# tlk00/BitMagic

Hardware: AMD Instinct MI355X
Metric: Gbits/s + % HBM roofline, 256-way fused AND+COUNT on 1B-bit vectors (higher is better)
Workload: dtype u64; 1 GPU; aggregator pipeline combine_and_sub counts-only: 256-way AND+COUNT, 256 x 1000000000-bit vectors in total, data set A (common 10% OR noise 10%: no early exit); vectors=256, bits_per_vector=1000000000, density_q16=6554, blocks_per_vector=15259, blocks_per_rank=15259, hbm_resident_bytes=32279432448

## Files before the change

bitmagic_amd/csrc/bmx_device.h:

```cpp
#pragma once
#include <hip/hip_runtime.h>
#include <stdint.h>

typedef uint8_t  u8;
typedef uint16_t u16;
typedef uint32_t u32;
typedef uint64_t u64;

#define GMETA(e) ((u32)((e) >> 48) & 0x1FFFu)
#define GMETA_NONE 0xFFFFFFFFu
#define BMX_DESC_KIND(d) ((u32)((d) & 3ull))
#define BMX_DESC_PTR(d)  ((d) & ~3ull)

typedef u32 u32x4 __attribute__((ext_vector_type(4)));
typedef const __attribute__((address_space(1))) u32x4* gcptr4;
typedef __attribute__((address_space(1))) u32x4* gptr4;
typedef const __attribute__((address_space(1))) u16* gcptr16;

template <int ROWS> struct Part { u32x4 r[ROWS]; };
typedef Part<8> Blk;

__device__ __forceinline__ gcptr4 as_gc4(u64 addr) { return (gcptr4)(uintptr_t)addr; }
__device__ __forceinline__ gcptr4 as_gc4(const void* p) { return (gcptr4)(uintptr_t)p; }
__device__ __forceinline__ gptr4 as_g4(void* p) { return (gptr4)(uintptr_t)p; }
__device__ __forceinline__ gcptr16 as_gc16(u64 addr) { return (gcptr16)(uintptr_t)(addr & 0x0000FFFFFFFFFFFFull); }

__device__ __forceinline__ u32 lane_id() { return threadIdx.x & 63u; }

__device__ __forceinline__ u64 uniform64(u64 v)
{
    u32 lo = __builtin_amdgcn_readfirstlane((u32)v);
    u32 hi = __builtin_amdgcn_readfirstlane((u32)(v >> 32));
    return ((u64)hi << 32) | lo;
}
__device__ __forceinline__ u32 uniform32(u32 v) { return __builtin_amdgcn_readfirstlane(v); }

__device__ __forceinline__ u32 wave_sum(u32 v)
{
#pragma unroll
    for (int o = 32; o > 0; o >>= 1) v += __shfl_xor(v, o, 64);
    return v;
}

__device__ __forceinline__ u32 wave_scan_incl(u32 v, u32 )
{
    v += (u32)__builtin_amdgcn_update_dpp(0, (int)v, 0x111, 0xf, 0xf, false);
    v += (u32)__builtin_amdgcn_update_dpp(0, (int)v, 0x112, 0xf, 0xf, false);
    v += (u32)__builtin_amdgcn_update_dpp(0, (int)v, 0x114, 0xf, 0xf, false);
    v += (u32)__builtin_amdgcn_update_dpp(0, (int)v, 0x118, 0xf, 0xf, false);
    v += (u32)__builtin_amdgcn_update_dpp(0, (int)v, 0x142, 0xa, 0xf, false);
    v += (u32)__builtin_amdgcn_update_dpp(0, (int)v, 0x143, 0xc, 0xf, false);
    return v;
}

template <int ROWS, bool NT>
__device__ __forceinline__ void part_load(Part<ROWS>& b, gcptr4 p, u32 lane)
{
#pragma unroll
    for (int i = 0; i < ROWS; ++i) {
        if constexpr (NT) b.r[i] = __builtin_nontemporal_load(p + i * 64 + lane);
        else b.r[i] = p[i * 64 + lane];
    }
}
template <int ROWS>
__device__ __forceinline__ bool part_is_zero(const Part<ROWS>& b)
{
    u32 v = 0;
#pragma unroll
    for (int i = 0; i < ROWS; ++i) v |= b.r[i].x | b.r[i].y | b.r[i].z | b.r[i].w;
    return __ballot(v != 0u) == 0ull;
}
template <int ROWS>
__device__ __forceinline__ bool part_is_ones(const Part<ROWS>& b)
{
    u32 v = ~0u;
#pragma unroll
    for (int i = 0; i < ROWS; ++i) v &= b.r[i].x & b.r[i].y & b.r[i].z & b.r[i].w;
    return __ballot(v != ~0u) == 0ull;
}

__device__ __forceinline__ void blk_load(Blk& b, gcptr4 p, u32 lane)
{
#pragma unroll
    for (int i = 0; i < 8; ++i) b.r[i] = p[i * 64 + lane];
}
__device__ __forceinline__ void blk_store(const Blk& b, gptr4 p, u32 lane)
{
#pragma unroll
    for (int i = 0; i < 8; ++i) p[i * 64 + lane] = b.r[i];
}
__device__ __forceinline__ void blk_fill(Blk& b, u32 v)
{
#pragma unroll
    for (int i = 0; i < 8; ++i) b.r[i] = (u32x4)(v);
}
__device__ __forceinline__ void blk_and(Blk& a, const Blk& b)
{
#pragma unroll
    for (int i = 0; i < 8; ++i) a.r[i] &= b.r[i];
}
__device__ __forceinline__ void blk_andn(Blk& a, const Blk& b)
{
#pragma unroll
    for (int i = 0; i < 8; ++i) a.r[i] &= ~b.r[i];
}
__device__ __forceinline__ void blk_or(Blk& a, const Blk& b)
{
#pragma unroll
    for (int i = 0; i < 8; ++i) a.r[i] |= b.r[i];
}
__device__ __forceinline__ void blk_xor(Blk& a, const Blk& b)
{
#pragma unroll
    for (int i = 0; i < 8; ++i) a.r[i] ^= b.r[i];
}
__device__ __forceinline__ void blk_op(int op, Blk& a, const Blk& b)
{
    switch (op) { case 0: blk_and(a, b); break; case 1: blk_or(a, b); break;
                  case 2: blk_xor(a, b); break; default: blk_andn(a, b); break; }
}
__device__ __forceinline__ u32 blk_lane_or(const Blk& b)
{
    u32 v = 0;
#pragma unroll
    for (int i = 0; i < 8; ++i) v |= b.r[i].x | b.r[i].y | b.r[i].z | b.r[i].w;
    return v;
}
__device__ __forceinline__ u32 blk_lane_and(const Blk& b)
{
    u32 v = ~0u;
#pragma unroll
    for (int i = 0; i < 8; ++i) v &= b.r[i].x & b.r[i].y & b.r[i].z & b.r[i].w;
    return v;
}
__device__ __forceinline__ bool blk_is_zero(const Blk& b) { return __ballot(blk_lane_or(b) != 0u) == 0ull; }
__device__ __forceinline__ bool blk_is_ones(const Blk& b) { return __ballot(blk_lane_and(b) != ~0u) == 0ull; }

__device__ __forceinline__ u32 blk_lane_popcount(const Blk& b)
{
    u32 c = 0;
#pragma unroll
    for (int i = 0; i < 8; ++i) {
        c += __popcll(((u64)b.r[i].y << 32) | b.r[i].x);
        c += __popcll(((u64)b.r[i].w << 32) | b.r[i].z);
    }
    return c;
}

__device__ __forceinline__ u32 blk_transitions(const Blk& b, Blk& t, u32 lane)
{
    u32 cnt = 0;
    u32 prev_row_last = 0;
#pragma unroll
    for (int i = 0; i < 8; ++i) {
        u32 w0 = b.r[i].x, w1 = b.r[i].y, w2 = b.r[i].z, w3 = b.r[i].w;
        u32 up = __shfl_up(w3, 1, 64) >> 31;
        u32 p0 = lane ? up : (i ? prev_row_last : (w0 & 1u));
        t.r[i].x = w0 ^ ((w0 << 1) | p0);
        t.r[i].y = w1 ^ ((w1 << 1) | (w0 >> 31));
        t.r[i].z = w2 ^ ((w2 << 1) | (w1 >> 31));
        t.r[i].w = w3 ^ ((w3 << 1) | (w2 >> 31));
        cnt += __popc(t.r[i].x) + __popc(t.r[i].y) + __popc(t.r[i].z) + __popc(t.r[i].w);
        prev_row_last = __shfl(w3, 63, 64) >> 31;
    }
    return cnt;
}

__device__ __forceinline__ u32 prefix_xor32(u32 x)
{
    x ^= x << 1; x ^= x << 2; x ^= x << 4; x ^= x << 8; x ^= x << 16;
    return x;
}

__device__ __forceinline__ void gap_decode_xor(gcptr16 g, u32* lds, Blk& out, u32 lane, u32 meta = GMETA_NONE)
{
    u32 len, sbit;
    if (meta != GMETA_NONE) { len = meta >> 1; sbit = meta & 1u; }
    else { u32 hdr = g[0]; len = hdr >> 3; sbit = hdr & 1u; }
    u32x4* l4 = reinterpret_cast<u32x4*>(lds);
#pragma unroll
    for (int i = 0; i < 8; ++i) l4[i * 64 + lane] = (u32x4)(0u);
    __builtin_amdgcn_fence(__ATOMIC_RELEASE, "wavefront");
    __builtin_amdgcn_wave_barrier();
    if (sbit && lane == 0) atomicXor(&lds[0], 1u);
    for (u32 kb = 1; kb < len; kb += 512u) {
        u32 e[8];
#pragma unroll
        for (int j = 0; j < 8; ++j) { u32 k = kb + (u32)j * 64u + lane; e[j] = k < len ? (u32)g[k] : 0xFFFFFFFFu; }
#pragma unroll
        for (int j = 0; j < 8; ++j) {
            if (e[j] != 0xFFFFFFFFu) { u32 p = e[j] + 1u; atomicXor(&lds[p >> 5], 1u << (p & 31u)); }
        }
    }
    __builtin_amdgcn_fence(__ATOMIC_ACQ_REL, "wavefront");
    __builtin_amdgcn_wave_barrier();
    u32 carry = 0;
#pragma unroll
    for (int i = 0; i < 8; ++i) {
        u32x4 t = l4[i * 64 + lane];
        u32 x0 = prefix_xor32(t.x), x1 = prefix_xor32(t.y), x2 = prefix_xor32(t.z), x3 = prefix_xor32(t.w);
        u64 b0 = __ballot((int)(x0 >> 31)), b1 = __ballot((int)(x1 >> 31));
        u64 b2 = __ballot((int)(x2 >> 31)), b3 = __ballot((int)(x3 >> 31));
        u32 below = __builtin_amdgcn_mbcnt_hi((u32)(b0 >> 32), __builtin_amdgcn_mbcnt_lo((u32)b0, 0));
        below = __builtin_amdgcn_mbcnt_hi((u32)(b1 >> 32), __builtin_amdgcn_mbcnt_lo((u32)b1, below));
        below = __builtin_amdgcn_mbcnt_hi((u32)(b2 >> 32), __builtin_amdgcn_mbcnt_lo((u32)b2, below));
        below = __builtin_amdgcn_mbcnt_hi((u32)(b3 >> 32), __builtin_amdgcn_mbcnt_lo((u32)b3, below));
        u32 c0 = (carry ^ below) & 1u;
        u32 c1 = c0 ^ (x0 >> 31), c2 = c1 ^ (x1 >> 31), c3 = c2 ^ (x2 >> 31);
        out.r[i].x = x0 ^ (0u - c0);
        out.r[i].y = x1 ^ (0u - c1);
        out.r[i].z = x2 ^ (0u - c2);
        out.r[i].w = x3 ^ (0u - c3);
        carry ^= (u32)(__popcll(b0) + __popcll(b1) + __popcll(b2) + __popcll(b3)) & 1u;
    }
    __builtin_amdgcn_wave_barrier();
}

enum { GAP_OR = 0, GAP_AND = 1, GAP_SUB = 2 };

template <int MODE>
__device__ __forceinline__ void lds_apply_edge(u32* lds, u32 w, u32 mask)
{
    if constexpr (MODE == GAP_OR) atomicOr(&lds[w], mask); else atomicAnd(&lds[w], ~mask);
}

template <int MODE>
__device__ __forceinline__ void lds_apply_run_edges(u32* lds, u32 s, u32 e)
{
    u32 wl = s >> 5, wr = e >> 5;
    u32 ml = ~0u << (s & 31u), mr = ~0u >> (31u - (e & 31u));
    if (wl == wr) lds_apply_edge<MODE>(lds, wl, ml & mr);
    else { lds_apply_edge<MODE>(lds, wl, ml); lds_apply_edge<MODE>(lds, wr, mr); }
}

template <int MODE>
__device__ __forceinline__ void gap_apply_lds_wave(gcptr16 g, u32* lds, u32 lane, u32 meta = GMETA_NONE)
{
    const u32 fill = (MODE == GAP_OR) ? ~0u : 0u;
    u32 len, sbit;
    if (meta != GMETA_NONE) { len = meta >> 1; sbit = meta & 1u; }
    else { u32 hdr = g[0]; len = hdr >> 3; sbit = hdr & 1u; }
    const u32 want = (MODE == GAP_AND) ? 0u : 1u;
    u32 k0 = (sbit == want) ? 1u : 2u;
    for (u32 kb = k0; kb <= len; kb += 512u) {
        u32 ee[4], ss[4];
#pragma unroll
        for (int j = 0; j < 4; ++j) {
            u32 k = kb + (u32)j * 128u + 2u * lane;
            u32 kk = k <= len ? k : len;
            ee[j] = (u32)g[kk]; ss[j] = (u32)g[kk - 1u];
        }
#pragma unroll
        for (int j = 0; j < 4; ++j) {
            u32 k = kb + (u32)j * 128u + 2u * lane;
            bool act = k <= len;
            ee[j] = act ? ee[j] : 0xFFFFFFFFu;
            ss[j] = act ? ((k == 1u) ? 0u : ss[j] + 1u) : 0u;
        }
#pragma unroll
        for (int j = 0; j < 4; ++j) {
            if (kb + (u32)j * 128u > len) break;
            bool act = ee[j] != 0xFFFFFFFFu;
            u32 s = ss[j], e = act ? ee[j] : 0u;
            if (act) lds_apply_run_edges<MODE>(lds, s, e);
            u32 wl = s >> 5, wr = e >> 5;
            u32 inner = (act && wr > wl + 1u) ? wr - wl - 1u : 0u;
            if (inner && inner <= 16u) for (u32 w = wl + 1u; w < wr; ++w) lds[w] = fill;
            u64 longm = __ballot(inner > 16u);
            while (longm) {
                u32 l = (u32)__builtin_ctzll(longm); longm &= longm - 1ull;
                u32 a = __builtin_amdgcn_readlane(wl, l) + 1u, b = __builtin_amdgcn_readlane(wr, l);
                for (u32 w = a + lane; w < b; w += 64u) lds[w] = fill;
            }
        }
    }
}

__device__ __forceinline__ void gap_decode(gcptr16 g, u32* lds, Blk& out, u32 lane, u32 meta = GMETA_NONE)
{
    u32x4* l4 = reinterpret_cast<u32x4*>(lds);
#pragma unroll
    for (int i = 0; i < 8; ++i) l4[i * 64 + lane] = (u32x4)(0u);
    __builtin_amdgcn_fence(__ATOMIC_RELEASE, "wavefront");
    __builtin_amdgcn_wave_barrier();
    gap_apply_lds_wave<GAP_OR>(g, lds, lane, meta);
    __builtin_amdgcn_fence(__ATOMIC_ACQ_REL, "wavefront");
    __builtin_amdgcn_wave_barrier();
#pragma unroll
    for (int i = 0; i < 8; ++i) out.r[i] = l4[i * 64 + lane];
    __builtin_amdgcn_wave_barrier();
}

template <int MODE>
__device__ __forceinline__ void gap_apply_chunk(u32* lds, const u32 x[5], u32 c, u32 len, bool odd_runs)
{
    const u32 fill = (MODE == GAP_OR) ? ~0u : 0u;
#pragma unroll
    for (int i = 0; i < 4; ++i) {
        u32 k, s, e;
        if (odd_runs) { k = 8u * c + 2u * i + 1u; s = (k == 1u) ? 0u : (x[i] & 0xFFFFu) + 1u; e = x[i] >> 16; }
        else          { k = 8u * c + 2u * i + 2u; s = (x[i] >> 16) + 1u; e = x[i + 1] & 0xFFFFu; }
        if (k <= len) {
            lds_apply_run_edges<MODE>(lds, s, e);
            for (u32 w = (s >> 5) + 1u; w < (e >> 5); ++w) lds[w] = fill;
        }
    }
}

template <int MODE>
__device__ __forceinline__ void gap_apply_lds_lane(gcptr16 g, u32* lds)
{
    const u32 want = (MODE == GAP_AND) ? 0u : 1u;
    gcptr4 g4 = (gcptr4)(uintptr_t)g;
    u32x4 c0 = g4[0], c1 = g4[1], c2 = g4[2], c3 = g4[3];
    u32 hdr = c0.x & 0xFFFFu;
    u32 len = hdr >> 3;
    bool odd_runs = (hdr & 1u) == want;
    u32 nchunks = (len + 8u) >> 3;
    { u32 x[5] = {c0.x, c0.y, c0.z, c0.w, c1.x}; gap_apply_chunk<MODE>(lds, x, 0, len, odd_runs); }
    if (nchunks > 1u) { u32 x[5] = {c1.x, c1.y, c1.z, c1.w, c2.x}; gap_apply_chunk<MODE>(lds, x, 1, len, odd_runs); }
    if (nchunks > 2u) { u32 x[5] = {c2.x, c2.y, c2.z, c2.w, c3.x}; gap_apply_chunk<MODE>(lds, x, 2, len, odd_runs); }
    if (nchunks > 3u) {
        u32x4 cur = c3;
        for (u32 c = 3; c < nchunks; ++c) {
            u32x4 nxt = (c + 1u < nchunks) ? g4[c + 1u] : cur;
            u32 x[5] = {cur.x, cur.y, cur.z, cur.w, nxt.x};
            gap_apply_chunk<MODE>(lds, x, c, len, odd_runs);
            cur = nxt;
        }
    }
}

struct GapHead { u32x4 c[4]; };

__device__ __forceinline__ void gap_head_fetch(GapHead& h, u64 gaddr, bool is_gap)
{
    gcptr4 g4 = (gcptr4)(uintptr_t)gaddr;
    if (is_gap) {
#pragma unroll
        for (int j = 0; j < 4; ++j) h.c[j] = g4[j];
    } else h.c[0].x = 0u;
}

__device__ __forceinline__ void gap_or_chunk_fast(u32* lds, const u32 x[5], u32 c, int lim, bool odd_runs)
{
#pragma unroll
    for (int i = 0; i < 4; ++i) {
        u32 y = odd_runs ? x[i] : __builtin_amdgcn_alignbit(x[i + 1], x[i], 16);
        u32 s = (y & 0xFFFFu) + 1u;
        if (c == 0u && i == 0) s = odd_runs ? 0u : s;
        u32 e = y >> 16;
        bool act = (int)(8u * c + 2u * (u32)i) <= lim;
        u32 wl = s >> 5, wr = e >> 5;
        u32 lo = 1u << (s & 31u), hi2 = 2u << (e & 31u);
        bool same = wl == wr;
        u32 m = (same ? hi2 : 0u) - lo;
        atomicOr(&lds[wl], act ? m : 0u);
        if (act && !same) {
            atomicOr(&lds[wr], hi2 - 1u);
            for (u32 w = wl + 1u; w < wr; ++w) lds[w] = ~0u;
        }
    }
}

__device__ __forceinline__ void gap_or_lane_fast(const GapHead& h, u64 gaddr, u32* lds)
{
    u32 hdr = h.c[0].x & 0xFFFFu;
    u32 len = hdr >> 3;
    bool odd_runs = (hdr & 1u) != 0u;
    int lim = (int)len - (odd_runs ? 1 : 2);
    u32 nchunks = (len + 8u) >> 3;
    { u32 x[5] = {h.c[0].x, h.c[0].y, h.c[0].z, h.c[0].w, h.c[1].x}; gap_or_chunk_fast(lds, x, 0, lim, odd_runs); }
    if (nchunks > 1u) { u32 x[5] = {h.c[1].x, h.c[1].y, h.c[1].z, h.c[1].w, h.c[2].x}; gap_or_chunk_fast(lds, x, 1, lim, odd_runs); }
    if (nchunks > 2u) { u32 x[5] = {h.c[2].x, h.c[2].y, h.c[2].z, h.c[2].w, h.c[3].x}; gap_or_chunk_fast(lds, x, 2, lim, odd_runs); }
    if (nchunks > 3u) {
        gcptr4 g4 = (gcptr4)(uintptr_t)gaddr;
        u32x4 cur = h.c[3];
        for (u32 c = 3; c < nchunks; ++c) {
            u32x4 nxt = (c + 1u < nchunks) ? g4[c + 1u] : cur;
            u32 x[5] = {cur.x, cur.y, cur.z, cur.w, nxt.x};
            gap_or_chunk_fast(lds, x, c, lim, odd_runs);
            cur = nxt;
        }
    }
}

__device__ __forceinline__ void gap_or_chunk_v2(u32* lds, const u32 x[5], u32 c, int lim)
{
#pragma unroll
    for (int i = 0; i < 4; ++i) {
        u32 y = __builtin_amdgcn_alignbit(x[i + 1], x[i], 16);
        u32 e = y >> 16;
        u32 d = e - (y & 0xFFFFu);
        bool act = (int)(8u * c + 2u * (u32)i) <= lim;
        bool single = d == 1u;
        atomicOr(&lds[e >> 5], (act && single) ? (1u << (e & 31u)) : 0u);
        if (act && !single) {
            u32 s = e - d + 1u;
            u32 wl = s >> 5, wr = e >> 5;
            u32 lo = 1u << (s & 31u), hi2 = 2u << (e & 31u);
            if (wl == wr) atomicOr(&lds[wl], hi2 - lo);
            else {
                atomicOr(&lds[wl], 0u - lo);
                atomicOr(&lds[wr], hi2 - 1u);
                for (u32 w = wl + 1u; w < wr; ++w) lds[w] = ~0u;
            }
        }
    }
}

__device__ __forceinline__ void gap_or_lane_v2(const GapHead& h, u64 gaddr, u32* lds)
{
    u32 hdr = h.c[0].x & 0xFFFFu;
    u32 len = hdr >> 3;
    bool odd_runs = (hdr & 1u) != 0u;
    if (__ballot(odd_runs) != 0ull) { gap_or_lane_fast(h, gaddr, lds); return; }
    int lim = (int)len - 2;
    u32 nchunks = (len + 8u) >> 3;
    { u32 x[5] = {h.c[0].x, h.c[0].y, h.c[0].z, h.c[0].w, h.c[1].x}; gap_or_chunk_v2(lds, x, 0, lim); }
    if (nchunks > 1u) { u32 x[5] = {h.c[1].x, h.c[1].y, h.c[1].z, h.c[1].w, h.c[2].x}; gap_or_chunk_v2(lds, x, 1, lim); }
    if (nchunks > 2u) { u32 x[5] = {h.c[2].x, h.c[2].y, h.c[2].z, h.c[2].w, h.c[3].x}; gap_or_chunk_v2(lds, x, 2, lim); }
    if (nchunks > 3u) {
        gcptr4 g4 = (gcptr4)(uintptr_t)gaddr;
        u32x4 cur = h.c[3];
        for (u32 c = 3; c < nchunks; ++c) {
            u32x4 nxt = (c + 1u < nchunks) ? g4[c + 1u] : cur;
            u32 x[5] = {cur.x, cur.y, cur.z, cur.w, nxt.x};
            gap_or_chunk_v2(lds, x, c, lim);
            cur = nxt;
        }
    }
}

__device__ __forceinline__ bool lds_blk_is_zero(const u32* lds, u32 lane)
{
    const u32x4* l4 = reinterpret_cast<const u32x4*>(lds);
    u32 v = 0;
#pragma unroll
    for (int i = 0; i < 8; ++i) { u32x4 t = l4[i * 64 + lane]; v |= t.x | t.y | t.z | t.w; }
    return __ballot(v != 0u) == 0ull;
}

__device__ __forceinline__ void blk_to_lds(const Blk& b, u32* lds, u32 lane)
{
    u32x4* l4 = reinterpret_cast<u32x4*>(lds);
#pragma unroll
    for (int i = 0; i < 8; ++i) l4[i * 64 + lane] = b.r[i];
    __builtin_amdgcn_fence(__ATOMIC_RELEASE, "wavefront");
    __builtin_amdgcn_wave_barrier();
}
__device__ __forceinline__ void blk_from_lds(Blk& b, const u32* lds, u32 lane)
{
    const u32x4* l4 = reinterpret_cast<const u32x4*>(lds);
#pragma unroll
    for (int i = 0; i < 8; ++i) b.r[i] = l4[i * 64 + lane];
}

__device__ __forceinline__ u32 lds_blk_popcount(const u32* lds, u32 lane)
{
    const u32x4* l4 = reinterpret_cast<const u32x4*>(lds);
    u32 c = 0;
#pragma unroll
    for (int i = 0; i < 8; ++i) {
        u32x4 t = l4[i * 64 + lane];
        c += (u32)__popc(t.x) + (u32)__popc(t.y) + (u32)__popc(t.z) + (u32)__popc(t.w);
    }
    return uniform32(wave_sum(c));
}

#define SPARSE_CAP 1024u
#define SPARSE_NONE 0xFFFFFFFFu

struct GapStage { u32x4 d[3]; };

__device__ __forceinline__ void gap_stage_load(GapStage& s, gcptr16 g, u32 hdr, u32 lane)
{
    gcptr4 g4 = (gcptr4)(uintptr_t)g;
    u32 nch = ((hdr >> 3) + 8u) >> 3;
    const u32x4 z = {0u, 0u, 0u, 0u};
#pragma unroll
    for (int j = 0; j < 3; ++j) { u32 c = lane + 64u * (u32)j; s.d[j] = c < nch ? g4[c] : z; }
}
__device__ __forceinline__ void gap_stage_store(const GapStage& s, u32* lds, u32 hdr, u32 lane)
{
    u32x4* l4 = reinterpret_cast<u32x4*>(lds);
    u32 nch = ((hdr >> 3) + 8u) >> 3;
#pragma unroll
    for (int j = 0; j < 3; ++j) { u32 c = lane + 64u * (u32)j; if (c < nch) l4[c] = s.d[j]; }
}

template <int MODE, int NJ>
__device__ __forceinline__ u32 sparse_test(u32 (&cand)[16], const u16* G, u32 hdr)
{
    u32 len = hdr >> 3, sbit = hdr & 1u;
    u32 k[NJ];
#pragma unroll
    for (int j = 0; j < NJ; ++j) k[j] = 0u;
    for (u32 step = 1u << (31 - __builtin_clz(len)); step; step >>= 1) {
#pragma unroll
        for (int j = 0; j < NJ; ++j) {
            u32 t = k[j] + step; t = t < len ? t : len;
            u32 v = G[t];
            k[j] = v < cand[j] ? t : k[j];
        }
    }
#pragma unroll
    for (int j = 0; j < NJ; ++j) {
        u32 bitv = (sbit ^ k[j]) & 1u;
        bool keep = (MODE == GAP_AND) ? (bitv != 0u) : (bitv == 0u);
        if (!keep) cand[j] = SPARSE_NONE;
    }
    u32 alive = 0;
#pragma unroll
    for (int j = 0; j < NJ; ++j) alive += (u32)__popcll(__ballot(cand[j] != SPARSE_NONE));
    return alive;
}

template <int MODE>
__device__ __forceinline__ bool gap_apply_sparse(const u64* __restrict__ plist_back, u32 i0, u32 n, u32* lds, u32 lane)
{
    u16* list = reinterpret_cast<u16*>(lds + 640);
    u32 cand[16];
    u32 total, nj;
    {
        Blk b; blk_from_lds(b, lds, lane);
        __builtin_amdgcn_fence(__ATOMIC_ACQ_REL, "wavefront");
        __builtin_amdgcn_wave_barrier();
        u32 cnt = blk_lane_popcount(b);
        u32 incl = wave_scan_incl(cnt, lane);
        total = uniform32(__shfl(incl, 63, 64));
        u32 off = incl - cnt;
#pragma unroll
        for (int i = 0; i < 8; ++i) {
            u32 ws[4] = {b.r[i].x, b.r[i].y, b.r[i].z, b.r[i].w};
#pragma unroll
            for (int c = 0; c < 4; ++c) {
                u32 w = ws[c];
                u32 base = ((u32)i * 256u + lane * 4u + (u32)c) << 5;
                while (w) { u32 bit = (u32)__builtin_ctz(w); w &= w - 1u; list[off++] = (u16)(base + bit); }
            }
        }
        __builtin_amdgcn_fence(__ATOMIC_ACQ_REL, "wavefront");
        __builtin_amdgcn_wave_barrier();
        nj = (total + 63u) >> 6;
#pragma unroll
        for (int j = 0; j < 16; ++j) {
            u32 idx = (u32)j * 64u + lane;
            cand[j] = idx < total ? (u32)list[idx] : SPARSE_NONE;
        }
    }
    const u16* G = reinterpret_cast<const u16*>(lds);
    u32 i = i0;
    gcptr16 g0 = as_gc16(uniform64(*(plist_back - i)));
    u32 h0 = uniform32((u32)g0[0]);
    GapStage cur; gap_stage_load(cur, g0, h0, lane);
    gcptr16 g1 = as_gc16(uniform64(*(plist_back - (i + 1u < n ? i + 1u : n - 1u))));
    u32 h1v = (u32)g1[0];
    for (; i < n; ++i) {
        u32 h1 = uniform32(h1v);
        GapStage nxt; gap_stage_load(nxt, g1, h1, lane);
        u32 i2 = i + 2u < n ? i + 2u : n - 1u;
        gcptr16 g2 = as_gc16(uniform64(*(plist_back - i2)));
        u32 h2v = (u32)g2[0];
        gap_stage_store(cur, lds, h0, lane);
        __builtin_amdgcn_fence(__ATOMIC_ACQ_REL, "wavefront");
        __builtin_amdgcn_wave_barrier();
        u32 alive;
        if (nj <= 1u) alive = sparse_test<MODE, 1>(cand, G, h0);
        else if (nj <= 2u) alive = sparse_test<MODE, 2>(cand, G, h0);
        else if (nj <= 3u) alive = sparse_test<MODE, 3>(cand, G, h0);
        else if (nj <= 4u) alive = sparse_test<MODE, 4>(cand, G, h0);
        else if (nj <= 6u) alive = sparse_test<MODE, 6>(cand, G, h0);
        else if (nj <= 8u) alive = sparse_test<MODE, 8>(cand, G, h0);
        else if (nj <= 12u) alive = sparse_test<MODE, 12>(cand, G, h0);
        else alive = sparse_test<MODE, 16>(cand, G, h0);
        if (alive == 0u) return true;
        if (((alive + 63u) >> 6) < nj) {
            u32 mine = 0;
#pragma unroll
            for (int j = 0; j < 16; ++j) mine += cand[j] != SPARSE_NONE ? 1u : 0u;
            u32 off = wave_scan_incl(mine, lane) - mine;
#pragma unroll
            for (int j = 0; j < 16; ++j) if (cand[j] != SPARSE_NONE) list[off++] = (u16)cand[j];
            __builtin_amdgcn_fence(__ATOMIC_ACQ_REL, "wavefront");
            __builtin_amdgcn_wave_barrier();
            nj = (alive + 63u) >> 6;
#pragma unroll
            for (int j = 0; j < 16; ++j) {
                u32 idx = (u32)j * 64u + lane;
                cand[j] = idx < alive ? (u32)list[idx] : SPARSE_NONE;
            }
        }
        __builtin_amdgcn_fence(__ATOMIC_ACQ_REL, "wavefront");
        __builtin_amdgcn_wave_barrier();
        cur = nxt; g0 = g1; h0 = h1; g1 = g2; h1v = h2v;
    }
    {
        u32x4* l4 = reinterpret_cast<u32x4*>(lds);
        const u32x4 z = {0u, 0u, 0u, 0u};
#pragma unroll
        for (int r = 0; r < 8; ++r) l4[r * 64 + lane] = z;
        __builtin_amdgcn_fence(__ATOMIC_ACQ_REL, "wavefront");
        __builtin_amdgcn_wave_barrier();
#pragma unroll
        for (int j = 0; j < 16; ++j)
            if (cand[j] != SPARSE_NONE) atomicOr(&lds[cand[j] >> 5], 1u << (cand[j] & 31u));
        __builtin_amdgcn_fence(__ATOMIC_ACQ_REL, "wavefront");
        __builtin_amdgcn_wave_barrier();
    }
    return false;
}

template <int MODE>
__device__ __forceinline__ bool gap_apply_list(const u64* __restrict__ plist_back, u32 n, u32* lds, u32 lane)
{
    const bool CHECK = MODE != GAP_OR;
    u32 head = n >= 32u ? 8u : n;
    u32 i = 0;
    if constexpr (CHECK) {
        if (n >= 2u) {
            u32 pop = lds_blk_popcount(lds, lane);
            if (pop == 0u) return true;
            if (pop <= SPARSE_CAP) return gap_apply_sparse<MODE>(plist_back, 0u, n, lds, lane);
        }
    }
    for (; i < head; ++i) {
        gap_apply_lds_wave<MODE>(as_gc16(uniform64(*(plist_back - i))), lds, lane);
        if constexpr (CHECK) {
            __builtin_amdgcn_fence(__ATOMIC_ACQ_REL, "wavefront");
            __builtin_amdgcn_wave_barrier();
            u32 pop = lds_blk_popcount(lds, lane);
            if (pop == 0u) return true;
            if (pop <= SPARSE_CAP && i + 2u < n) return gap_apply_sparse<MODE>(plist_back, i + 1u, n, lds, lane);
        }
    }
    if (i < n) {
        u64 p = i + lane < n ? *(plist_back - (i + lane)) : 0ull;
        for (; i < n; i += 64u) {
            u64 pn = i + 64u + lane < n ? *(plist_back - (i + 64u + lane)) : 0ull;
            if (i + lane < n) gap_apply_lds_lane<MODE>(as_gc16(p), lds);
            p = pn;
            if constexpr (CHECK) {
                __builtin_amdgcn_fence(__ATOMIC_ACQ_REL, "wavefront");
                __builtin_amdgcn_wave_barrier();
                u32 pop = lds_blk_popcount(lds, lane);
                if (pop == 0u) return true;
                if (pop <= SPARSE_CAP && i + 64u + 2u <= n)
                    return gap_apply_sparse<MODE>(plist_back, i + 64u, n, lds, lane);
            }
        }
    }
    __builtin_amdgcn_fence(__ATOMIC_ACQ_REL, "wavefront");
    __builtin_amdgcn_wave_barrier();
    return false;
}

__device__ __forceinline__ u32 gap_lane_popcount(gcptr16 g, u32 lane, u32 meta = GMETA_NONE)
{
    u32 len, s;
    if (meta != GMETA_NONE) { len = meta >> 1; s = meta & 1u; }
    else { u32 hdr = g[0]; len = hdr >> 3; s = hdr & 1u; }
    u32 c = 0;
    for (u32 k = 1 + lane; k <= len; k += 64) {
        u32 e = g[k], pe = g[k - 1];
        bool one = (s ^ ((k - 1u) & 1u)) != 0u;
        c += one ? ((k == 1u) ? e + 1u : e - pe) : 0u;
    }
    return c;
}

__device__ __forceinline__ u64 mix64(u64 x)
{
    x ^= x >> 30; x *= 0xBF58476D1CE4E5B9ull;
    x ^= x >> 27; x *= 0x94D049BB133111EBull;
    x ^= x >> 31;
    return x;
}
__device__ __forceinline__ u64 gen_word64(u64 seed, u32 vec_id, u64 w64, u32 d)
{
    if (d >= 65536u) return ~0ull;
    u64 base = seed ^ ((u64)vec_id * 0x9E3779B97F4A7C15ull);
    u64 acc = 0;
#pragma unroll
    for (u32 k = 0; k < 16; ++k) {
        u64 r = mix64(base + (w64 * 16u + k) * 0xD6E8FEB86659FD93ull);
        acc = ((d >> k) & 1u) ? (acc | r) : (acc & r);
    }
    return acc;
}

__device__ __forceinline__ u64 readlane64(u64 v, u32 l)
{
    u32 lo = __builtin_amdgcn_readlane((u32)v, l);
    u32 hi = __builtin_amdgcn_readlane((u32)(v >> 32), l);
    return ((u64)hi << 32) | lo;
}

template <int U, bool NT, int OPK, int ROWS = 8>
__device__ __forceinline__ bool pipe_chain(Part<ROWS>& acc, const u64* __restrict__ plist, u32 n, u32 lane, u32 poff = 0u)
{
    if (n == 0) return false;
    u64 pn[U];
    auto fetch = [&](u32 k) {
#pragma unroll
        for (int u = 0; u < U; ++u) pn[u] = plist[k + u < n ? k + u : n - 1u];
    };
    auto issue = [&](Part<ROWS>* buf) {
#pragma unroll
        for (int u = 0; u < U; ++u) part_load<ROWS, NT>(buf[u], as_gc4(uniform64(pn[u])) + poff, lane);
    };
    auto consume = [&](Part<ROWS>* buf) {
#pragma unroll
        for (int u = 0; u < U; ++u)
#pragma unroll
            for (int i = 0; i < ROWS; ++i) {
                if constexpr (OPK == 0) acc.r[i] &= buf[u].r[i];
                else if constexpr (OPK == 1) acc.r[i] &= ~buf[u].r[i];
                else acc.r[i] |= buf[u].r[i];
            }
        if constexpr (OPK == 2) return part_is_ones<ROWS>(acc); else return part_is_zero<ROWS>(acc);
    };
    Part<ROWS> A[U], B[U];
    u32 k = U;
    fetch(0);
    issue(A);
    fetch(k);
    bool zero;
    do {
        issue(B); fetch(k + U);
        bool z1 = consume(A);
        issue(A); fetch(k + 2 * U);
        bool z2 = consume(B);
        zero = z1 | z2;
        k += 2 * U;
    } while (!zero && k < n + U);
    return zero;
}
```

bitmagic_amd/csrc/bmx_kernels.h:

```cpp
#pragma once
#include "bmx_device.h"

#define DESC_MAKE(ptr, kind) ((u64)(uintptr_t)(ptr) | ((u64)(kind) << 62))
#define DESC_K(d) ((u32)((d) >> 62))
#define DESC_P(d) ((d) & 0x0000FFFFFFFFFFFFull)
#define DESC_MAKE_GAP(ptr, len, sbit) (DESC_MAKE(ptr, K_GAP) | ((u64)((((u32)(len)) << 1) | ((u32)(sbit) & 1u)) << 48))
enum { K_NULL = 0, K_FULL = 1, K_BIT = 2, K_GAP = 3 };

#define ROW_EMPTY 1ull
#define ROW_FULL  2ull
#define ROW_ONES  4ull

struct BlockStat { u32 pop; u32 runs; u32 first; u32 kind; };

__global__ __launch_bounds__(256)
void k_generate(u64 seed, u32 vec_id, int with_common, u32 d, u64 nbits, u64* __restrict__ out, u64 nwords64, u64 word0)
{
    u64 i = (u64)blockIdx.x * blockDim.x + threadIdx.x;
    u64 stride = (u64)gridDim.x * blockDim.x;
    for (; i < nwords64; i += stride) {
        u64 w = word0 + i;
        u64 v = gen_word64(seed, vec_id, w, d);
        if (with_common) v |= gen_word64(seed, 0xFFFFFFFFu, w, d);
        u64 bit0 = w * 64u;
        if (bit0 >= nbits) v = 0;
        else if (nbits - bit0 < 64u) v &= (~0ull) >> (64u - (nbits - bit0));
        out[i] = v;
    }
}

__global__ __launch_bounds__(256)
void k_block_stats(const uint4* __restrict__ raw, u32 nblocks, int optimize, BlockStat* __restrict__ st)
{
    u32 lane = lane_id();
    u32 nb = uniform32(blockIdx.x * 4u + (threadIdx.x >> 6));
    if (nb >= nblocks) return;
    Blk b, t;
    blk_load(b, as_gc4(raw + (size_t)nb * 512u), lane);
    u32 pop = wave_sum(blk_lane_popcount(b));
    u32 runs = 1u + wave_sum(blk_transitions(b, t, lane));
    u32 first = __shfl(b.r[0].x, 0, 64) & 1u;
    if (lane == 0) {
        u32 kind = !optimize ? K_BIT
                 : (runs == 1u) ? (first ? K_FULL : K_NULL)
                 : (runs < 1276u ? K_GAP : K_BIT);
        st[nb] = BlockStat{pop, runs, first, kind};
    }
}

#define SCAN_PER 16u
#define SCAN_LAYOUT_PER 8u
__global__ __launch_bounds__(1024)
void k_scan_layout(const BlockStat* __restrict__ st, u32 nblocks, u32* __restrict__ offs, u64* __restrict__ totals)
{
    __shared__ u32 sm[32];
    __shared__ u32 kcnt[4];
    u32 tid = threadIdx.x, lane = tid & 63u, w = tid >> 6;
    if (tid < 4) kcnt[tid] = 0;
    __syncthreads();
    u32 carry_bit = 0, carry_gap = 0;
    u32 kc[4] = {0, 0, 0, 0};
    const uint4* st4 = reinterpret_cast<const uint4*>(st);
    for (u32 base = 0; base < nblocks; base += 1024u * SCAN_LAYOUT_PER) {
        u32 nb0 = base + w * (64u * SCAN_LAYOUT_PER) + lane;
        u32 kind[SCAN_LAYOUT_PER], e[SCAN_LAYOUT_PER];
        uint4 x[SCAN_LAYOUT_PER];
#pragma unroll
        for (u32 i = 0; i < SCAN_LAYOUT_PER; ++i) {
            u32 nb = nb0 + i * 64u;
            x[i] = nb < nblocks ? st4[nb] : make_uint4(0u, 0u, 0u, 0xFFu);
        }
        u32 run_b = 0, run_g = 0;
#pragma unroll
        for (u32 i = 0; i < SCAN_LAYOUT_PER; ++i) {
            kind[i] = x[i].w;
            u32 vg = kind[i] == K_GAP ? ((x[i].y + 1u + 7u) & ~7u) : 0u;
            u64 mb = __ballot(kind[i] == K_BIT), mg = __ballot(kind[i] == K_GAP);
            kc[K_BIT] += (u32)__popcll(mb); kc[K_GAP] += (u32)__popcll(mg);
            kc[K_FULL] += (u32)__popcll(__ballot(kind[i] == K_FULL)); kc[K_NULL] += (u32)__popcll(__ballot(kind[i] == K_NULL));
            u32 ig = wave_scan_incl(vg, lane);
            u32 eb = run_b + __builtin_amdgcn_mbcnt_hi((u32)(mb >> 32), __builtin_amdgcn_mbcnt_lo((u32)mb, 0u));
            e[i] = kind[i] == K_BIT ? eb : run_g + ig - vg;
            run_b += (u32)__popcll(mb); run_g += __shfl(ig, 63, 64);
        }
        if (lane == 0) { sm[w] = run_b; sm[16 + w] = run_g; }
        __syncthreads();
        u32 ob = carry_bit, og = carry_gap, tb = 0, tg = 0;
#pragma unroll
        for (u32 i = 0; i < 16; ++i) { u32 a = sm[i], b = sm[16 + i]; if (i < w) { ob += a; og += b; } tb += a; tg += b; }
        __syncthreads();
#pragma unroll
        for (u32 i = 0; i < SCAN_LAYOUT_PER; ++i) {
            u32 nb = nb0 + i * 64u;
            if (nb < nblocks) offs[nb] = kind[i] == K_BIT ? ob + e[i] : (kind[i] == K_GAP ? og + e[i] : 0u);
        }
        carry_bit += tb; carry_gap += tg;
    }
#pragma unroll
    for (int k = 0; k < 4; ++k)
        if (lane == 0 && kc[k]) atomicAdd(&kcnt[k], kc[k]);
    __syncthreads();
    if (tid == 0) { totals[0] = carry_bit; totals[1] = carry_gap; }
    if (tid < 4) totals[2 + tid] = kcnt[tid];
}

__global__ __launch_bounds__(256)
void k_emit_blocks(const uint4* __restrict__ raw, u32 nblocks, const BlockStat* __restrict__ st,
                   const u32* __restrict__ offs, uint4* __restrict__ bit_slab, u16* __restrict__ gap_slab,
                   u64* __restrict__ desc)
{
    u32 lane = lane_id();
    u32 nb = uniform32(blockIdx.x * 4u + (threadIdx.x >> 6));
    if (nb >= nblocks) return;
    u32 kind = uniform32(st[nb].kind);
    if (kind == K_NULL || kind == K_FULL) { if (lane == 0) desc[nb] = DESC_MAKE(0, kind); return; }
    Blk b;
    blk_load(b, as_gc4(raw + (size_t)nb * 512u), lane);
    if (kind == K_BIT) {
        uint4* dst = bit_slab + (size_t)offs[nb] * 512u;
        blk_store(b, as_g4(dst), lane);
        if (lane == 0) desc[nb] = DESC_MAKE(dst, K_BIT);
        return;
    }
    u16* g = gap_slab + offs[nb];
    Blk t;
    (void)blk_transitions(b, t, lane);
    u32 len = uniform32(st[nb].runs);
    u32 idx_base = 1u;
#pragma unroll
    for (int i = 0; i < 8; ++i) {
        u32 c = __popc(t.r[i].x) + __popc(t.r[i].y) + __popc(t.r[i].z) + __popc(t.r[i].w);
        u32 incl = wave_scan_incl(c, lane);
        u32 idx = idx_base + incl - c;
        u32 wbase = (u32)i * 256u + lane * 4u;
        u32 tw[4] = {t.r[i].x, t.r[i].y, t.r[i].z, t.r[i].w};
#pragma unroll
        for (int j = 0; j < 4; ++j) {
            u32 m = tw[j];
            while (m) {
                u32 k = __builtin_ctz(m); m &= m - 1u;
                g[idx++] = (u16)((wbase + j) * 32u + k - 1u);
            }
        }
        idx_base += __shfl(incl, 63, 64);
    }
    if (lane == 0) {
        u32 level = len <= 124u ? 0u : len <= 252u ? 1u : len <= 508u ? 2u : 3u;
        g[0] = (u16)((len << 3) | (level << 1) | st[nb].first);
        g[len] = 65535u;
        desc[nb] = DESC_MAKE_GAP(g, len, st[nb].first);
    }
    if (lane >= 1u && lane <= 7u && len + lane < ((len + 1u + 7u) & ~7u)) g[len + lane] = 0xFFFFu;
}

__global__ __launch_bounds__(256)
void k_gap_repack(const u16* __restrict__ raw, const u32* __restrict__ src_off, const u64* __restrict__ desc,
                  u32 nblocks, u64* __restrict__ err)
{
    u32 lane = lane_id();
    u32 nb = uniform32(blockIdx.x * 4u + (threadIdx.x >> 6));
    if (nb >= nblocks) return;
    u64 d = uniform64(desc[nb]);
    if (DESC_K(d) != K_GAP) return;
    const u16* src = raw + src_off[nb];
    u16* dst = (u16*)(uintptr_t)DESC_P(d);
    u32 len = GMETA(d) >> 1;
    u32 padded = (len + 1u + 7u) & ~7u;
    bool bad = false;
    for (u32 k = lane; k < padded; k += 64u) {
        u32 cur = k <= len ? (u32)src[k] : 0xFFFFu;
        if (k >= 2u && k <= len && (u32)src[k - 1u] >= cur) bad = true;
        if (k == len && cur != 65535u) bad = true;
        dst[k] = (u16)cur;
    }
    if (__ballot(bad) != 0ull && lane == 0) atomicOr(reinterpret_cast<unsigned long long*>(err), 1ull);
}

__device__ __forceinline__ void blk_from_desc(u64 d, Blk& b, u32* lds, u32 lane)
{
    u32 k = DESC_K(d);
    if (k == K_BIT) blk_load(b, as_gc4(DESC_P(d)), lane);
    else if (k == K_GAP) gap_decode(as_gc16(DESC_P(d)), lds, b, lane, GMETA(d));
    else blk_fill(b, k == K_FULL ? ~0u : 0u);
}

#define COUNT_SLOTS 64u
#define COUNT_SLOT_STRIDE 16u
__device__ __forceinline__ void count_fanin(u32 wave_count, u64* __restrict__ slots, u32 lane, u32 wave)
{
    __shared__ u32 part[16];
    u32 nw = blockDim.x >> 6;
    if (lane == 0) part[wave] = wave_count;
    __syncthreads();
    if (threadIdx.x == 0) {
        u64 t = 0;
        for (u32 i = 0; i < nw; ++i) t += part[i];
        if (t) atomicAdd(reinterpret_cast<unsigned long long*>(slots + (blockIdx.x % COUNT_SLOTS) * COUNT_SLOT_STRIDE), (unsigned long long)t);
    }
}
__global__ __launch_bounds__(64)
void k_sum_slots(u64* __restrict__ slots, u64* __restrict__ out)
{
    u32 lane = threadIdx.x;
    u64 v = slots[lane * COUNT_SLOT_STRIDE];
    slots[lane * COUNT_SLOT_STRIDE] = 0;
    for (int o = 32; o > 0; o >>= 1) v += __shfl_xor(v, o, 64);
    if (lane == 0) *out = v;
}

struct FoldOut { u64* slots; u32* done; u64* out; };
#define FOLD_DONE_WORDS (32u * (COUNT_SLOTS + 1u))

#if defined(__HIP_DEVICE_COMPILE__) && !defined(__GFX9__)
#error "fold_publish orders relaxed atomics with s_waitcnt vmcnt(0): valid on the gfx9 family (gfx90a/gfx942/gfx950) only"
#endif
__device__ __forceinline__ bool fold_publish(u64 v, FoldOut f)
{
    u32 s_ = blockIdx.x % COUNT_SLOTS;
    u64* slot = f.slots + s_ * COUNT_SLOT_STRIDE;
    if (v) {
        (void)__hip_atomic_fetch_add(slot, v, __ATOMIC_RELAXED, __HIP_MEMORY_SCOPE_AGENT);
        asm volatile("s_waitcnt vmcnt(0)" ::: "memory");
    }
    u32 expect = gridDim.x / COUNT_SLOTS + (s_ < gridDim.x % COUNT_SLOTS ? 1u : 0u);
    u32 k = __hip_atomic_fetch_add(f.done + 32u * (1u + s_), 1u, __ATOMIC_RELAXED, __HIP_MEMORY_SCOPE_AGENT);
    if (k != expect - 1u) return false;
    __hip_atomic_store(f.done + 32u * (1u + s_), 0u, __ATOMIC_RELAXED, __HIP_MEMORY_SCOPE_AGENT);
    u32 used = gridDim.x < COUNT_SLOTS ? gridDim.x : COUNT_SLOTS;
    asm volatile("s_waitcnt vmcnt(0)" ::: "memory");
    u32 g = __hip_atomic_fetch_add(f.done, 1u, __ATOMIC_RELAXED, __HIP_MEMORY_SCOPE_AGENT);
    if (g != used - 1u) return false;
    __hip_atomic_store(f.done, 0u, __ATOMIC_RELAXED, __HIP_MEMORY_SCOPE_AGENT);
    return true;
}

__device__ __forceinline__ void count_fanin_fold(u32 wave_count, FoldOut f, u32 lane, u32 wave)
{
    __shared__ u32 part[16];
    u32 nw = blockDim.x >> 6;
    if (lane == 0) part[wave] = wave_count;
    __syncthreads();
    if (wave == 0) {
        u32 folder = 0;
        if (lane == 0) {
            u64 t = 0;
            for (u32 i = 0; i < nw; ++i) t += part[i];
            folder = fold_publish(t, f) ? 1u : 0u;
        }
        if (__shfl(folder, 0, 64)) {
            u64 v = __hip_atomic_exchange(f.slots + lane * COUNT_SLOT_STRIDE, 0ull, __ATOMIC_RELAXED, __HIP_MEMORY_SCOPE_AGENT);
            for (int o = 32; o > 0; o >>= 1) v += __shfl_xor(v, o, 64);
            if (lane == 0) __hip_atomic_store(f.out, v, __ATOMIC_RELAXED, __HIP_MEMORY_SCOPE_SYSTEM);
        }
    }
}

__device__ __forceinline__ void kind_fanin_fold_packed(u64 wave_kinds, FoldOut f, u32 lane, u32 wave, u64* extra = nullptr)
{
    __shared__ u64 wk[16];
    u32 nw = blockDim.x >> 6;
    if (lane == 0) wk[wave] = wave_kinds;
    __syncthreads();
    if (wave == 0) {
        u32 folder = 0;
        if (lane == 0) {
            u64 t = 0;
            for (u32 i = 0; i < nw; ++i) t += wk[i];
            folder = fold_publish(t, f) ? 1u : 0u;
        }
        if (__shfl(folder, 0, 64)) {
            u64 v = __hip_atomic_exchange(f.slots + lane * COUNT_SLOT_STRIDE, 0ull, __ATOMIC_RELAXED, __HIP_MEMORY_SCOPE_AGENT);
#pragma unroll
            for (int k = 0; k < 4; ++k) {
                u32 c = (u32)((v >> (16 * k)) & 0xFFFFull);
                c = wave_sum(c);
                if (lane == 0) __hip_atomic_store(f.out + k, (u64)c, __ATOMIC_RELAXED, __HIP_MEMORY_SCOPE_SYSTEM);
            }
            if (extra && lane == 0) {
                const u64 cur = __hip_atomic_exchange(extra, 0ull, __ATOMIC_RELAXED, __HIP_MEMORY_SCOPE_AGENT);
                __hip_atomic_store(f.out + 4, cur, __ATOMIC_RELAXED, __HIP_MEMORY_SCOPE_SYSTEM);
            }
        }
    }
}
__device__ __forceinline__ void kind_fanin_fold(u32 kind , FoldOut f, u32 lane, u32 wave)
{
    kind_fanin_fold_packed(kind < 4u ? 1ull << (16u * kind) : 0ull, f, lane, wave);
}

__global__ __launch_bounds__(256)
void k_vec_count(const u64* __restrict__ desc, u32 nblocks, FoldOut fold)
{
    u32 lane = lane_id(), wave = threadIdx.x >> 6;
    u32 nb = uniform32(blockIdx.x * 4u + wave);
    u32 c = 0;
    if (nb < nblocks) {
        u64 d = uniform64(desc[nb]);
        u32 k = DESC_K(d);
        if (k == K_FULL) c = 65536u;
        else if (k == K_BIT) { Blk b; blk_load(b, as_gc4(DESC_P(d)), lane); c = wave_sum(blk_lane_popcount(b)); }
        else if (k == K_GAP) c = wave_sum(gap_lane_popcount(as_gc16(DESC_P(d)), lane, GMETA(d)));
    }
    count_fanin_fold(c, fold, lane, wave);
}

__global__ __launch_bounds__(256)
void k_vec_expand(const u64* __restrict__ desc, u32 nblocks, u32 nblocks_out, uint4* __restrict__ out)
{
    __shared__ u32 lds[4 * 2048];
    u32 lane = lane_id(), wave = threadIdx.x >> 6;
    u32 nb = uniform32(blockIdx.x * 4u + wave);
    if (nb >= nblocks_out) return;
    u64 d = nb < nblocks ? uniform64(desc[nb]) : 0ull;
    Blk b;
    if (DESC_K(d) == K_GAP) gap_decode_xor(as_gc16(DESC_P(d)), lds + wave * 2048u, b, lane, GMETA(d));
    else blk_from_desc(d, b, lds + wave * 2048u, lane);
    blk_store(b, as_g4(out + (size_t)nb * 512u), lane);
}

struct PipeOperands {
    const u64* const* desc;
    const u32* nblocks;
    const u32* and_off; const u32* and_n;
    const u32* sub_off; const u32* sub_n;
    const u32* row_off;
};

__device__ __forceinline__ bool sort_operands(const u64* const* __restrict__ desc, const u32* __restrict__ nblocks,
                                              u32 off, u32 n, u32 c, u32 kill, u64* __restrict__ region,
                                              u32& nbit, u32& ngap, u32 lane)
{
    bool killed = false;
    nbit = 0; ngap = 0;
    for (u32 base = 0; base < n; base += 64u) {
        u32 k = base + lane;
        bool valid = k < n;
        u32 op = off + (valid ? k : n - 1u);
        u32 nb = nblocks[op];
        const u64* dp = desc[op];
        u64 d = dp[c < nb ? c : 0u];
        if (!valid || c >= nb) d = 0ull;
        u32 kd = valid ? DESC_K(d) : 4u;
        if (__ballot(valid && kd == kill) != 0ull) killed = true;
        u64 bit_m = __ballot(kd == K_BIT), gap_m = __ballot(kd == K_GAP);
        u64 lt = (1ull << lane) - 1ull;
        if (kd == K_BIT) region[nbit + (u32)__popcll(bit_m & lt)] = DESC_P(d);
        if (kd == K_GAP) region[n - 1u - (ngap + (u32)__popcll(gap_m & lt))] = d & 0x3FFFFFFFFFFFFFFFull;
        nbit += (u32)__popcll(bit_m); ngap += (u32)__popcll(gap_m);
    }
    return killed;
}

__global__ __launch_bounds__(256)
void k_pipe_sort(PipeOperands po, u32 ngroups, u32 ncols, u32 col_stride, u64* __restrict__ dmat)
{
    u32 lane = lane_id();
    u64 wid = (u64)blockIdx.x * (blockDim.x >> 6) + (threadIdx.x >> 6);
    if (wid >= (u64)ncols * ngroups) return;
    u32 c = (u32)(wid / ngroups), g = (u32)(wid - (u64)c * ngroups);
    u64* row = dmat + (size_t)c * col_stride + po.row_off[g];
    u32 na = po.and_n[g], ns = po.sub_n[g];
    u32 ao = po.and_off[g], so = po.sub_off[g];
    u32 nbit = 0, ngap = 0, sbit = 0, sgap = 0;
    bool empty = (na == 0);
    if (na && sort_operands(po.desc, po.nblocks, ao, na, c, K_NULL, row + 2, nbit, ngap, lane)) empty = true;
    if (!empty && ns && sort_operands(po.desc, po.nblocks, so, ns, c, K_FULL, row + 2 + na, sbit, sgap, lane)) empty = true;
    u64 flags = 0;
    if (empty) flags = ROW_EMPTY;
    else if (!nbit && !ngap) { if (!sbit && !sgap) flags = ROW_FULL; else flags = ROW_ONES; }
    else if (!nbit) flags = ROW_ONES;
    if (lane == 0) {
        row[0] = (u64)nbit | ((u64)ngap << 16) | ((u64)sbit << 32) | ((u64)sgap << 48);
        row[1] = flags;
    }
}

__device__ __forceinline__ u32 xcd_remap(u32 b, u32 nwg)
{
    u32 q = nwg >> 3, rem = nwg & 7u;
    u32 x = b & 7u, i = b >> 3;
    return x * q + (x < rem ? x : rem) + i;
}

template <int U>
__global__ __launch_bounds__(256)
void k_pipe_counts(const u64* __restrict__ dmat, const u32* __restrict__ row_off,
                   const u32* __restrict__ and_n, const u32* __restrict__ sub_n, u32 col_stride,
                   u32 ngroups, u32 col_from, u32 nitems, int xcd_swz, u64* __restrict__ counts)
{
    extern __shared__ u32 lds_dyn[];
    u32 lane = lane_id(), wave = threadIdx.x >> 6;
    u32 bid = xcd_swz ? xcd_remap(blockIdx.x, gridDim.x) : blockIdx.x;
    u32 item = uniform32(bid * 4u + wave);
    if (item >= nitems) return;
    u32 c = item / ngroups, g = item - c * ngroups;
    const u64* row = dmat + (size_t)(col_from + c) * col_stride + row_off[g];
    u64 hdr = uniform64(row[0]), flags = uniform64(row[1]);
    if (flags & ROW_EMPTY) return;
    if (flags & ROW_FULL) { if (lane == 0) atomicAdd(reinterpret_cast<unsigned long long*>(&counts[g]), 65536ull); return; }
    u32 nba = (u32)(hdr & 0xFFFFu), nga = (u32)((hdr >> 16) & 0xFFFFu);
    u32 nbs = (u32)((hdr >> 32) & 0xFFFFu), ngs = (u32)(hdr >> 48);
    u32 na = uniform32(and_n[g]), ns = uniform32(sub_n[g]);
    const u64* pa = row + 2;
    const u64* ps = pa + na;
    u32* lds = lds_dyn + wave * 2048u;

    Blk acc;
    blk_fill(acc, ~0u);
    if (pipe_chain<U, true, 0>(acc, pa, nba, lane)) return;
    if (pipe_chain<U, true, 1>(acc, ps, nbs, lane)) return;
    if (nga | ngs) {
        blk_to_lds(acc, lds, lane);
        if (nga && gap_apply_list<GAP_AND>(pa + na - 1u, nga, lds, lane)) return;
        if (ngs && gap_apply_list<GAP_SUB>(ps + ns - 1u, ngs, lds, lane)) return;
        blk_from_lds(acc, lds, lane);
    }
    u32 cnt = wave_sum(blk_lane_popcount(acc));
    if (lane == 0 && cnt) atomicAdd(reinterpret_cast<unsigned long long*>(&counts[g]), (unsigned long long)cnt);
}

template <int U, bool NT, int WG = 256, int ROWS = 8>
__global__ __launch_bounds__(WG)
void k_pipe_counts_bits2(const u64* __restrict__ dmat, const u32* __restrict__ row_off,
                         const u32* __restrict__ and_n, u32 col_stride,
                         u32 ngroups, u32 col_from, u32 nitems, int xcd_swz, u64* __restrict__ counts)
{
    constexpr u32 PARTS = 8 / ROWS;
    u32 lane = lane_id(), wave = threadIdx.x >> 6, wpb = blockDim.x >> 6;
    u32 bid = xcd_swz ? xcd_remap(blockIdx.x, gridDim.x) : blockIdx.x;
    u32 item = uniform32(bid * wpb + wave);
    if (item >= nitems) return;
    u32 part = item % PARTS, cg = item / PARTS;
    u32 c = cg / ngroups, g = cg - c * ngroups;
    const u64* row = dmat + (size_t)(col_from + c) * col_stride + row_off[g];
    u64 hdr = uniform64(row[0]), flags = uniform64(row[1]);
    if (flags & ROW_EMPTY) return;
    if (flags & ROW_FULL) { if (lane == 0) atomicAdd(reinterpret_cast<unsigned long long*>(&counts[g]), (unsigned long long)(65536u / PARTS)); return; }
    u32 nba = (u32)(hdr & 0xFFFFu), nbs = (u32)((hdr >> 32) & 0xFFFFu);
    u32 na = uniform32(and_n[g]);
    const u64* pa = row + 2;
    const u64* ps = pa + na;
    const u32 poff = part * ROWS * 64u;
    Part<ROWS> acc;
#pragma unroll
    for (int i = 0; i < ROWS; ++i) acc.r[i] = (u32x4)(~0u);
    if (pipe_chain<U, NT, 0, ROWS>(acc, pa, nba, lane, poff)) return;
    if (pipe_chain<U, NT, 1, ROWS>(acc, ps, nbs, lane, poff)) return;
    u32 cnt = 0;
#pragma unroll
    for (int i = 0; i < ROWS; ++i) {
        cnt += __popcll(((u64)acc.r[i].y << 32) | acc.r[i].x);
        cnt += __popcll(((u64)acc.r[i].w << 32) | acc.r[i].z);
    }
    cnt = wave_sum(cnt);
    if (lane == 0 && cnt) atomicAdd(reinterpret_cast<unsigned long long*>(&counts[g]), (unsigned long long)cnt);
}

#ifdef BMX_DIAG
template <int AUX>
__global__ __launch_bounds__(256)
void k_diag_stream_read_buf(const uint4* __restrict__ buf, u64 nblocks8k, u32 blocks_per_wave, int pattern, int xcd_swz, u64* __restrict__ sink)
{
    u32 lane = lane_id();
    u32 bid = xcd_swz ? xcd_remap(blockIdx.x, gridDim.x) : blockIdx.x;
    u64 w = (u64)bid * (blockDim.x >> 6) + (threadIdx.x >> 6);
    u64 nwaves = nblocks8k / blocks_per_wave;
    if (w >= nwaves) return;
    u64 b0 = pattern ? w : w * blocks_per_wave;
    u64 step = pattern ? nwaves : 1;
    u32x4 acc = (u32x4)(0u);
    for (u32 j = 0; j < blocks_per_wave; ++j) {
        u64 addr = uniform64((u64)(uintptr_t)(buf + (b0 + j * step) * 512u));
        __amdgpu_buffer_rsrc_t r = __builtin_amdgcn_make_buffer_rsrc((void*)(uintptr_t)addr, 0, 8192, 0x00020000);
#pragma unroll
        for (int i = 0; i < 8; ++i) acc |= __builtin_amdgcn_raw_buffer_load_b128(r, (int)(i * 1024 + lane * 16), 0, AUX);
    }
    if ((acc.x | acc.y | acc.z | acc.w) == 0x12345678u) sink[0] = 1;
}

#endif

__global__ __launch_bounds__(256)
void k_pipe_bytes(const u64* __restrict__ dmat, const u32* __restrict__ row_off, const u32* __restrict__ and_n,
                  const u32* __restrict__ sub_n, u32 col_stride, u32 ngroups, u32 col_from, u32 nitems,
                  u64* __restrict__ total)
{
    u64 tid = (u64)blockIdx.x * blockDim.x + threadIdx.x;
    u64 bytes = 0;
    if (tid < nitems) {
        u32 c = (u32)(tid / ngroups), g = (u32)(tid - (u64)c * ngroups);
        const u64* row = dmat + (size_t)(col_from + c) * col_stride + row_off[g];
        u64 hdr = row[0], flags = row[1];
        if (!(flags & (ROW_EMPTY | ROW_FULL))) {
            u32 nba = (u32)(hdr & 0xFFFFu), nga = (u32)((hdr >> 16) & 0xFFFFu);
            u32 nbs = (u32)((hdr >> 32) & 0xFFFFu), ngs = (u32)(hdr >> 48);
            bytes = (u64)(nba + nbs) * 8192ull;
            const u64* pa = row + 2; const u64* ps = pa + and_n[g];
            for (u32 i = 0; i < nga; ++i) bytes += 2ull * ((as_gc16(pa[and_n[g] - 1u - i])[0] >> 3) + 1u);
            for (u32 i = 0; i < ngs; ++i) bytes += 2ull * ((as_gc16(ps[sub_n[g] - 1u - i])[0] >> 3) + 1u);
        }
    }
    __shared__ u64 s[256];
    s[threadIdx.x] = bytes; __syncthreads();
    for (u32 o = 128; o > 0; o >>= 1) { if (threadIdx.x < o) s[threadIdx.x] += s[threadIdx.x + o]; __syncthreads(); }
    if (threadIdx.x == 0 && s[0]) atomicAdd(reinterpret_cast<unsigned long long*>(total), (unsigned long long)s[0]);
}

#ifdef BMX_DIAG
template <bool NT>
__global__ __launch_bounds__(256)
void k_diag_stream_read(const uint4* __restrict__ buf, u64 nblocks8k, u32 blocks_per_wave, int pattern, int xcd_swz, u64* __restrict__ sink)
{
    u32 lane = lane_id();
    u32 bid = xcd_swz ? xcd_remap(blockIdx.x, gridDim.x) : blockIdx.x;
    u64 w = (u64)bid * (blockDim.x >> 6) + (threadIdx.x >> 6);
    u64 nwaves = nblocks8k / blocks_per_wave;
    if (w >= nwaves) return;
    u64 b0 = pattern ? w : w * blocks_per_wave;
    u64 step = pattern ? nwaves : 1;
    u32x4 acc = (u32x4)(0u);
    for (u32 j = 0; j < blocks_per_wave; ++j) {
        Part<8> t;
        part_load<8, NT>(t, as_gc4(buf + (b0 + j * step) * 512u), lane);
#pragma unroll
        for (int i = 0; i < 8; ++i) acc |= t.r[i];
    }
    if ((acc.x | acc.y | acc.z | acc.w) == 0x12345678u) sink[0] = 1;
}
#endif
```

Baseline: 56010 Gbit/s.

## Add sparse-accumulator probe path that loads only rows with live bits

The AND / AND-NOT chain now tracks how many wave lanes still hold nonzero accumulator bits. Once that count falls to a threshold, it stops the full pipelined chain and switches to a probe loop that loads only rows whose accumulator is still nonzero, so it fetches less HBM data for sparse intersections. The cost is a ballot plus popcount on every pipeline step and a serialized first load batch before the overlapped loop starts. On inputs where the intersection stays dense, the probe path never triggers and these costs remain.

```diff
diff --git a/bitmagic_amd/csrc/bmx_device.h b/bitmagic_amd/csrc/bmx_device.h
--- a/bitmagic_amd/csrc/bmx_device.h
+++ b/bitmagic_amd/csrc/bmx_device.h
@@ -61,6 +61,14 @@
         if constexpr (NT) b.r[i] = __builtin_nontemporal_load(p + i * 64 + lane);
         else b.r[i] = p[i * 64 + lane];
     }
+}
+template <int ROWS>
+__device__ __forceinline__ u32 part_live_lanes(const Part<ROWS>& b)
+{
+    u32 v = 0;
+#pragma unroll
+    for (int i = 0; i < ROWS; ++i) v |= b.r[i].x | b.r[i].y | b.r[i].z | b.r[i].w;
+    return (u32)__builtin_popcountll(__ballot(v != 0u));
 }
 template <int ROWS>
 __device__ __forceinline__ bool part_is_zero(const Part<ROWS>& b)
@@ -696,10 +704,19 @@
     return ((u64)hi << 32) | lo;
 }
 
-template <int U, bool NT, int OPK, int ROWS = 8>
-__device__ __forceinline__ bool pipe_chain(Part<ROWS>& acc, const u64* __restrict__ plist, u32 n, u32 lane, u32 poff = 0u)
-{
-    if (n == 0) return false;
+#define PIPE_SPARSE_LANES 16u
+
+struct PipeState {
+    u32 next;
+    u32 live;
+};
+
+template <int U, bool NT, int OPK, int ROWS = 8, bool SP = false>
+__device__ __forceinline__ auto pipe_chain(Part<ROWS>& acc, const u64* __restrict__ plist, u32 n, u32 lane, u32 poff = 0u)
+{
+    static_assert(!SP || OPK != 2, "the sparse state exists for AND / AND-NOT only");
+    if constexpr (SP) { if (n == 0) return PipeState{0u, 64u}; }
+    else { if (n == 0) return false; }
     u64 pn[U];
     auto fetch = [&](u32 k) {
 #pragma unroll
@@ -709,7 +726,7 @@
 #pragma unroll
         for (int u = 0; u < U; ++u) part_load<ROWS, NT>(buf[u], as_gc4(uniform64(pn[u])) + poff, lane);
     };
-    auto consume = [&](Part<ROWS>* buf) {
+    auto apply = [&](Part<ROWS>* buf) {
 #pragma unroll
         for (int u = 0; u < U; ++u)
 #pragma unroll
@@ -718,21 +735,81 @@
                 else if constexpr (OPK == 1) acc.r[i] &= ~buf[u].r[i];
                 else acc.r[i] |= buf[u].r[i];
             }
+    };
+    auto consume = [&](Part<ROWS>* buf) {
+        apply(buf);
         if constexpr (OPK == 2) return part_is_ones<ROWS>(acc); else return part_is_zero<ROWS>(acc);
     };
     Part<ROWS> A[U], B[U];
     u32 k = U;
     fetch(0);
-    issue(A);
-    fetch(k);
-    bool zero;
-    do {
-        issue(B); fetch(k + U);
-        bool z1 = consume(A);
-        issue(A); fetch(k + 2 * U);
-        bool z2 = consume(B);
-        zero = z1 | z2;
-        k += 2 * U;
-    } while (!zero && k < n + U);
-    return zero;
-}
+    if constexpr (SP) {
+        issue(A);
+        fetch(k);
+        apply(A);
+        u32 live = part_live_lanes<ROWS>(acc);
+        if (live <= PIPE_SPARSE_LANES || n <= (u32)U) return PipeState{n < (u32)U ? n : (u32)U, live};
+        issue(A);
+        k = 2 * U;
+        fetch(k);
+        bool sparse;
+        do {
+            issue(B); fetch(k + U);
+            apply(A);
+            const bool s1 = part_live_lanes<ROWS>(acc) <= PIPE_SPARSE_LANES;
+            issue(A); fetch(k + 2 * U);
+            apply(B);
+            live = part_live_lanes<ROWS>(acc);
+            sparse = s1 | (live <= PIPE_SPARSE_LANES);
+            k += 2 * U;
+        } while (!sparse && k < n + U);
+        return PipeState{k - U < n ? k - U : n, live};
+    } else {
+        issue(A);
+        fetch(k);
+        bool zero;
+        do {
+            issue(B); fetch(k + U);
+            bool z1 = consume(A);
+            issue(A); fetch(k + 2 * U);
+            bool z2 = consume(B);
+            zero = z1 | z2;
+            k += 2 * U;
+        } while (!zero && k < n + U);
+        return zero;
+    }
+}
+
+template <bool NT, int OPK, int ROWS>
+__device__ __forceinline__ bool pipe_probe(Part<ROWS>& acc, const u64* __restrict__ plist, u32 k, u32 n, u32 lane, u32 poff)
+{
+    constexpr int T = 2;
+    for (; k < n; k += T) {
+        gcptr4 p[T];
+#pragma unroll
+        for (int t = 0; t < T; ++t) p[t] = as_gc4(uniform64(plist[k + t < n ? k + t : n - 1u])) + poff;
+        Part<ROWS> buf[T];
+#pragma unroll
+        for (int i = 0; i < ROWS; ++i) {
+            const bool on = (acc.r[i].x | acc.r[i].y | acc.r[i].z | acc.r[i].w) != 0u;
+#pragma unroll
+            for (int t = 0; t < T; ++t) buf[t].r[i] = (u32x4)(0u);
+            if (on) {
+#pragma unroll
+                for (int t = 0; t < T; ++t) {
+                    if constexpr (NT) buf[t].r[i] = __builtin_nontemporal_load(p[t] + i * 64 + lane);
+                    else buf[t].r[i] = p[t][i * 64 + lane];
+                }
+            }
+        }
+#pragma unroll
+        for (int t = 0; t < T; ++t)
+#pragma unroll
+            for (int i = 0; i < ROWS; ++i) {
+                if constexpr (OPK == 0) acc.r[i] &= buf[t].r[i];
+                else acc.r[i] &= ~buf[t].r[i];
+            }
+        if (part_is_zero<ROWS>(acc)) return true;
+    }
+    return false;
+}
diff --git a/bitmagic_amd/csrc/bmx_kernels.h b/bitmagic_amd/csrc/bmx_kernels.h
--- a/bitmagic_amd/csrc/bmx_kernels.h
+++ b/bitmagic_amd/csrc/bmx_kernels.h
@@ -444,8 +444,17 @@
     Part<ROWS> acc;
 #pragma unroll
     for (int i = 0; i < ROWS; ++i) acc.r[i] = (u32x4)(~0u);
-    if (pipe_chain<U, NT, 0, ROWS>(acc, pa, nba, lane, poff)) return;
-    if (pipe_chain<U, NT, 1, ROWS>(acc, ps, nbs, lane, poff)) return;
+    PipeState st = pipe_chain<U, NT, 0, ROWS, true>(acc, pa, nba, lane, poff);
+    u32 and_next = st.next, sub_next = 0u;
+    if (st.live > PIPE_SPARSE_LANES) {
+        st = pipe_chain<U, NT, 1, ROWS, true>(acc, ps, nbs, lane, poff);
+        sub_next = st.next;
+    }
+    if (st.live == 0u) return;
+    if (st.live <= PIPE_SPARSE_LANES) {
+        if (pipe_probe<NT, 0, ROWS>(acc, pa, and_next, nba, lane, poff)) return;
+        if (pipe_probe<NT, 1, ROWS>(acc, ps, sub_next, nbs, lane, poff)) return;
+    }
     u32 cnt = 0;
 #pragma unroll
     for (int i = 0; i < ROWS; ++i) {
```

After: 55510 Gbit/s. About the same (-0.9%).
